# Kier73/Adaptive-Matrix-Solver

Measured on AMD Instinct MI355X. Metric: candidate-steps/sec, n=4096 dense eig pop=256, 1/2/4/8 GPUs vs CPU ref, higher is better.
Workload: dtype f64; 1 GPU; n=4096 dense non-Hermitian eig (complex128 Ginibre/sqrt(n)), initial_num_candidates=256, direct-LU InverseIterateSolver path; n=4096, pop=256, device= (gfx950:sramecc+:xnack-)

## Files before the change

adaptive_matrix_solver_amd/csrc/zgemm.hip:

```cpp
#include "common.h"
#include <cstdlib>

#ifndef MAUS_WC
#define MAUS_WC 8
#endif

namespace {

struct TCol { int x, y, z; };
__device__ __forceinline__ long tile_off(long rows, int col) { return ((long)(col >> 6) * rows << 6) + (col & 63); }

template <int BM, int BN, int BK, int WM, int WN, int BLAY, bool CONJA, bool CONJB, bool PIPE, int MINW, bool M3 = false, bool TILED = false>
__global__ void __launch_bounds__(64 * WM * WN, MINW)
zgemm_kernel(int M, int N, int K,
             const c128* __restrict__ Ag, long lda, long strideA,
             const c128* __restrict__ Bg, long ldb, long strideB,
             c128* __restrict__ Cg, long ldc, long strideC,
             double alpha, int beta, int tiles_n, int nwg,
             const int* __restrict__ a_rows, const int* __restrict__ c_rows, long rows_stride, TCol tcol)
{
    static_assert(!TILED || (BLAY == 0 && !CONJA && !CONJB && BK == 16), "tiled operands: plain layout, K-tiles of 16");
    constexpr int NT = 64 * WM * WN;
    constexpr int WTM = BM / WM, WTN = BN / WN;
    constexpr int MB = WTM / 16, NB = WTN / 16;
    constexpr int LDA_S = BM, LDB_S = BN;
    constexpr int A_PER = BM * BK / NT, B_PER = BN * BK / NT;
    static_assert(A_PER * NT == BM * BK && B_PER * NT == BN * BK, "tile/threads mismatch");

    constexpr int TILE_S = BK * LDA_S + BK * LDB_S;
    __shared__ c128 smem[(PIPE ? 2 : 1) * TILE_S];

    int bid = blockIdx.x;
    {
        int q = nwg >> 3, r = nwg & 7, xcd = bid & 7, idx = bid >> 3;
        bid = (xcd < r ? xcd * (q + 1) : r * (q + 1) + (xcd - r) * q) + idx;
    }
#ifndef MAUS_WC
#define MAUS_WC 8
#endif
    constexpr int WC = MAUS_WC;
    const int tiles_m = nwg / tiles_n;
    const int full = tiles_m * WC;
    int cb = bid / full, rem = bid - cb * full, wl = WC;
    const int ncb = (tiles_n + WC - 1) / WC;
    if (cb >= ncb - 1) { cb = ncb - 1; rem = bid - cb * full; wl = tiles_n - cb * WC; }
    const int tm = rem / wl, tn = cb * WC + (rem - tm * wl);
    const int m0 = tm * BM, n0 = tn * BN;
    const long batch = blockIdx.y;
    const c128* A = Ag + batch * strideA;
    const c128* B = Bg + batch * strideB;
    c128* C = Cg + batch * strideC;
    if (a_rows) a_rows += batch * rows_stride;
    if (c_rows) c_rows += batch * rows_stride;

    const int tid = threadIdx.x, lane = tid & 63, wave = tid >> 6;
    const int wm = wave / WN, wn = wave - wm * WN;

    d4 cre[MB][NB], cim[MB][NB], c3[M3 ? MB : 1][M3 ? NB : 1];
#pragma unroll
    for (int i = 0; i < MB; ++i)
#pragma unroll
        for (int j = 0; j < NB; ++j) {
            cre[i][j] = (d4){0, 0, 0, 0}; cim[i][j] = (d4){0, 0, 0, 0};
            if (M3) c3[i][j] = (d4){0, 0, 0, 0};
        }

    c128 ra[A_PER], rb[B_PER];

    const bool KEDGE = (K % BK) != 0;
    const c128* pa[A_PER];
    const c128* pb[B_PER];
#pragma unroll
    for (int i = 0; i < A_PER; ++i) {
        int r = tid / BK + i * (NT / BK);
        int gm = min(m0 + r, M - 1);
        pa[i] = A + (long)(a_rows ? a_rows[gm] : gm) * (TILED ? 64 : lda);
    }
#pragma unroll
    for (int i = 0; i < B_PER; ++i) {
        if (BLAY == 0) { int gn = min(n0 + tid % BN, N - 1); pb[i] = B + (TILED ? tile_off(ldb, tcol.z + gn) + (long)tcol.y * 64 : (long)gn); }
        else { int gn = min(n0 + tid / BK + i * (NT / BK), N - 1); pb[i] = B + (long)gn * ldb; }
    }
    const long ldb_e = TILED ? 64 : ldb;
    if (BLAY == 0) {
#pragma unroll
        for (int i = 0; i < B_PER; ++i) pb[i] += (long)(tid / BN + i * (NT / BN)) * ldb_e;
    }
    int kload = 0;
    auto load_tiles = [&](int k0) {
        kload = k0;
        const long ta = TILED ? tile_off(lda, tcol.x + k0) : 0;
#pragma unroll
        for (int i = 0; i < A_PER; ++i) {
            int gk = k0 + (tid & (BK - 1));
            if (TILED) ra[i] = pa[i][ta + (tid & (BK - 1))];
            else ra[i] = pa[i][KEDGE ? min(gk, K - 1) : gk];
        }
#pragma unroll
        for (int i = 0; i < B_PER; ++i) {
            if (BLAY == 0) {
                const int kr = tid / BN + i * (NT / BN);
                if (!KEDGE || TILED) rb[i] = pb[i][(long)k0 * ldb_e];
                else rb[i] = pb[i][(long)(min(k0 + kr, K - 1) - kr) * ldb];
            } else {
                int gk = k0 + (tid & (BK - 1));
                rb[i] = pb[i][KEDGE ? min(gk, K - 1) : gk];
            }
        }
    };
    auto store_tiles = [&](int buf) {
        c128* As = smem + buf * TILE_S;
        c128* Bs = As + BK * LDA_S;
#pragma unroll
        for (int i = 0; i < A_PER; ++i) {
            int k = tid & (BK - 1), r = tid / BK + i * (NT / BK);
            c128 v = ra[i];
            if (KEDGE && kload + k >= K) v = cmake(0.0, 0.0);
            if (CONJA) v.y = -v.y;
            As[k * LDA_S + (r ^ (k & 7))] = v;
        }
        if (BLAY == 0) {
#pragma unroll
            for (int i = 0; i < B_PER; ++i) {
                int n = tid % BN, k = tid / BN + i * (NT / BN);
                c128 v = rb[i];
                if (KEDGE && kload + k >= K) v = cmake(0.0, 0.0);
                if (CONJB) v.y = -v.y;
                Bs[k * LDB_S + (n ^ (k & 7))] = v;
            }
        } else {
#pragma unroll
            for (int i = 0; i < B_PER; ++i) {
                int k = tid & (BK - 1), r = tid / BK + i * (NT / BK);
                c128 v = rb[i];
                if (KEDGE && kload + k >= K) v = cmake(0.0, 0.0);
                if (CONJB) v.y = -v.y;
                Bs[k * LDB_S + (r ^ (k & 7))] = v;
            }
        }
    };

    const int nkt = (K + BK - 1) / BK;
    constexpr int KSTEPS = BK / 4;
    c128 fa[2][MB], fb[2][NB];
    auto read_frags = [&](int buf, int kk, int slot) {
        const c128* As = smem + buf * TILE_S;
        const c128* Bs = As + BK * LDA_S;
        const int krow = kk * 4 + (lane >> 4);
#pragma unroll
        for (int i = 0; i < MB; ++i) fa[slot][i] = As[krow * LDA_S + ((wm * WTM + i * 16 + (lane & 15)) ^ (krow & 7))];
#pragma unroll
        for (int j = 0; j < NB; ++j) fb[slot][j] = Bs[krow * LDB_S + ((wn * WTN + j * 16 + (lane & 15)) ^ (krow & 7))];
    };
    auto mfma_group = [&](int slot) {
        if (M3) {
            double as[MB], bs[NB];
#pragma unroll
            for (int i = 0; i < MB; ++i) as[i] = fa[slot][i].x + fa[slot][i].y;
#pragma unroll
            for (int j = 0; j < NB; ++j) bs[j] = fb[slot][j].x + fb[slot][j].y;
#pragma unroll
            for (int i = 0; i < MB; ++i)
#pragma unroll
                for (int j = 0; j < NB; ++j) {
                    cre[i][j] = __builtin_amdgcn_mfma_f64_16x16x4f64(fa[slot][i].x, fb[slot][j].x, cre[i][j], 0, 0, 0);
                    cim[i][j] = __builtin_amdgcn_mfma_f64_16x16x4f64(fa[slot][i].y, fb[slot][j].y, cim[i][j], 0, 0, 0);
                    c3[i][j] = __builtin_amdgcn_mfma_f64_16x16x4f64(as[i], bs[j], c3[i][j], 0, 0, 0);
                }
        } else {
#pragma unroll
            for (int i = 0; i < MB; ++i)
#pragma unroll
                for (int j = 0; j < NB; ++j) {
                    cre[i][j] = __builtin_amdgcn_mfma_f64_16x16x4f64(fa[slot][i].x, fb[slot][j].x, cre[i][j], 0, 0, 0);
                    cim[i][j] = __builtin_amdgcn_mfma_f64_16x16x4f64(fa[slot][i].x, fb[slot][j].y, cim[i][j], 0, 0, 0);
                }
#pragma unroll
            for (int i = 0; i < MB; ++i)
#pragma unroll
                for (int j = 0; j < NB; ++j) {
                    cre[i][j] = __builtin_amdgcn_mfma_f64_16x16x4f64(fa[slot][i].y, fb[slot][j].y, cre[i][j], 0, 0, 1);
                    cim[i][j] = __builtin_amdgcn_mfma_f64_16x16x4f64(fa[slot][i].y, fb[slot][j].x, cim[i][j], 0, 0, 0);
                }
        }
    };

    if (PIPE) {
        load_tiles(0);
        store_tiles(0);
        if (nkt > 1) load_tiles(BK);
        __syncthreads();
        for (int kt = 0; kt < nkt; ++kt) {
            const int buf = kt & 1;
            read_frags(buf, 0, 0);
#pragma unroll
            for (int kk = 0; kk < KSTEPS; ++kk) {
                if (kk + 1 < KSTEPS) read_frags(buf, kk + 1, (kk + 1) & 1);
                if (kk == 0 && kt + 1 < nkt) store_tiles(buf ^ 1);
                if (kk == 0 && kt + 2 < nkt) load_tiles((kt + 2) * BK);
                __builtin_amdgcn_sched_barrier(0);
                mfma_group(kk & 1);
                __builtin_amdgcn_sched_barrier(0);
            }
            __syncthreads();
        }
    } else {
        load_tiles(0);
        for (int kt = 0; kt < nkt; ++kt) {
            __syncthreads();
            store_tiles(0);
            __syncthreads();
            if (kt + 1 < nkt) load_tiles((kt + 1) * BK);
            read_frags(0, 0, 0);
#pragma unroll
            for (int kk = 0; kk < KSTEPS; ++kk) {
                if (kk + 1 < KSTEPS) read_frags(0, kk + 1, (kk + 1) & 1);
                mfma_group(kk & 1);
            }
        }
    }

#pragma unroll
    for (int i = 0; i < MB; ++i)
#pragma unroll
        for (int j = 0; j < NB; ++j) {
            const int gn = n0 + wn * WTN + j * 16 + (lane & 15);
            c128 cold[4];
            long off[4];
#pragma unroll
            for (int r = 0; r < 4; ++r) {
                const int gm = m0 + wm * WTM + i * 16 + (lane >> 4) + 4 * r;
                const int cm = min(gm, M - 1), cn = min(gn, N - 1);
                off[r] = TILED ? (long)(c_rows ? c_rows[cm] : cm) * 64 + tile_off(ldc, tcol.z + cn)
                               : (long)(c_rows ? c_rows[cm] : cm) * ldc + cn;
                cold[r] = cmake(0.0, 0.0);
                if (beta) cold[r] = C[off[r]];
            }
#pragma unroll
            for (int r = 0; r < 4; ++r) {
                const int gm = m0 + wm * WTM + i * 16 + (lane >> 4) + 4 * r;
                if (gm < M && gn < N) {
                    const double vr = M3 ? cre[i][j][r] - cim[i][j][r] : cre[i][j][r];
                    const double vi = M3 ? (c3[i][j][r] - cre[i][j][r]) - cim[i][j][r] : cim[i][j][r];
                    C[off[r]] = cmake(alpha * vr + cold[r].x, alpha * vi + cold[r].y);
                }
            }
        }
}

template <int NST, int MINW, int MB, int NB, bool TILED = false, int BLAY = 0, bool CONJA = false, bool CONJB = false>
__global__ void __launch_bounds__(256, MINW)
zgemm3m_dma_kernel(int M, int N, int K,
                   const c128* __restrict__ Ag, long lda, long strideA,
                   const c128* __restrict__ Bg, long ldb, long strideB,
                   c128* __restrict__ Cg, long ldc, long strideC,
                   double alpha, int beta, int tiles_n, int nwg,
                   const int* __restrict__ a_rows, const int* __restrict__ c_rows, long rows_stride, TCol tcol)
{
    constexpr int WN = 2, BM = 2 * 16 * MB, BN = WN * 16 * NB, BKS = 8;
    constexpr int A_ST = BM * BKS, B_ST = BKS * BN;
    constexpr int A_PW = BM / 32;
    constexpr int B_PW = BN / 32;
    constexpr int DMA_PW = A_PW + B_PW;
    __shared__ c128 smem[NST * (A_ST + B_ST)];

    int bid = blockIdx.x;
    {
        int q = nwg >> 3, r = nwg & 7, xcd = bid & 7, idx = bid >> 3;
        bid = (xcd < r ? xcd * (q + 1) : r * (q + 1) + (xcd - r) * q) + idx;
    }
    constexpr int WC = MAUS_WC;
    const int tiles_m = nwg / tiles_n;
    const int full = tiles_m * WC;
    int cb = bid / full, rem = bid - cb * full, wl = WC;
    const int ncb = (tiles_n + WC - 1) / WC;
    if (cb >= ncb - 1) { cb = ncb - 1; rem = bid - cb * full; wl = tiles_n - cb * WC; }
    const int tm = rem / wl, tn = cb * WC + (rem - tm * wl);
    const int m0 = tm * BM, n0 = tn * BN;
    const long batch = blockIdx.y;
    const c128* A = Ag + batch * strideA;
    const c128* B = Bg + batch * strideB;
    c128* C = Cg + batch * strideC;
    if (a_rows) a_rows += batch * rows_stride;
    if (c_rows) c_rows += batch * rows_stride;

    const int tid = threadIdx.x, lane = tid & 63, wave = tid >> 6;
    const int wm = wave / WN, wn = wave - wm * WN;

    const c128* srcA[A_PW];
#pragma unroll
    for (int j = 0; j < A_PW; ++j) {
        const int r = (A_PW * wave + j) * 8 + (lane >> 3);
        const int kk = (lane & 7) ^ ((r >> 1) & 7);
        const int gm = min(m0 + r, M - 1);
        srcA[j] = A + (long)(a_rows ? a_rows[gm] : gm) * (TILED ? 64 : lda) + kk;
    }
    static_assert(!(TILED && BLAY), "tiled operands: plain layout only");
    const c128* srcB[B_PW];
    const long ldb_e = TILED ? 64 : ldb;
#pragma unroll
    for (int j = 0; j < B_PW; ++j) {
        if (BLAY == 0) {
            const int e = (B_PW * wave + j) * 64 + lane;
            const int gn = min(n0 + (e % BN), N - 1);
            srcB[j] = B + (long)(e / BN) * ldb_e + (TILED ? tile_off(ldb, tcol.z + gn) + (long)tcol.y * 64 : (long)gn);
        } else {
            const int r = (B_PW * wave + j) * 8 + (lane >> 3);
            const int kk = (lane & 7) ^ ((r >> 1) & 7);
            srcB[j] = B + (long)min(n0 + r, N - 1) * ldb + kk;
        }
    }

    auto issue = [&](int st, int k0) {
        c128* As = smem + st * (A_ST + B_ST);
        c128* Bs = As + A_ST;
        const long ta = TILED ? tile_off(lda, tcol.x + k0) : (long)k0;
#pragma unroll
        for (int j = 0; j < A_PW; ++j)
            __builtin_amdgcn_global_load_lds((const void*)(srcA[j] + ta), (__attribute__((address_space(3))) void*)(As + (A_PW * wave + j) * 64), 16, 0, 0);
#pragma unroll
        for (int j = 0; j < B_PW; ++j)
            __builtin_amdgcn_global_load_lds((const void*)(srcB[j] + (BLAY ? (long)k0 : (long)k0 * ldb_e)), (__attribute__((address_space(3))) void*)(Bs + (B_PW * wave + j) * 64), 16, 0, 0);
    };

    d4 cre[MB][NB], cim[MB][NB], c3[MB][NB];
#pragma unroll
    for (int i = 0; i < MB; ++i)
#pragma unroll
        for (int j = 0; j < NB; ++j) { cre[i][j] = (d4){0, 0, 0, 0}; cim[i][j] = (d4){0, 0, 0, 0}; c3[i][j] = (d4){0, 0, 0, 0}; }

    const int nst = K / BKS;
#pragma unroll
    for (int s = 0; s < NST - 1; ++s) if (s < nst) issue(s, s * BKS);

    const int arow0 = wm * 16 * MB + (lane & 15);
    const int bcol0 = wn * 16 * NB + (lane & 15);
    const int q = lane >> 4;
    for (int t = 0; t < nst; ++t) {
        if (NST >= 3 && t + NST - 2 < nst) asm volatile("s_waitcnt vmcnt(%0)" :: "n"((NST - 2) * DMA_PW) : "memory");
        else asm volatile("s_waitcnt vmcnt(0)" ::: "memory");
        __builtin_amdgcn_s_barrier();
        asm volatile("" ::: "memory");
        const c128* As = smem + (t % NST) * (A_ST + B_ST);
        const c128* Bs = As + A_ST;
        c128 fa[2][MB], fb[2][NB];
#pragma unroll
        for (int ks = 0; ks < 2; ++ks) {
            const int k = ks * 4 + q;
#pragma unroll
            for (int i = 0; i < MB; ++i) {
                const int r = arow0 + i * 16;
                fa[ks][i] = As[r * BKS + (k ^ ((r >> 1) & 7))];
            }
#pragma unroll
            for (int j = 0; j < NB; ++j) {
                const int cn = bcol0 + j * 16;
                fb[ks][j] = BLAY ? Bs[cn * BKS + (k ^ ((cn >> 1) & 7))] : Bs[k * BN + cn];
            }
        }
        if (t + NST - 1 < nst) issue((t + NST - 1) % NST, (t + NST - 1) * BKS);
#pragma unroll
        for (int ks = 0; ks < 2; ++ks) {
            double as[MB], bs[NB];
#pragma unroll
            for (int i = 0; i < MB; ++i) as[i] = CONJA ? fa[ks][i].x - fa[ks][i].y : fa[ks][i].x + fa[ks][i].y;
#pragma unroll
            for (int j = 0; j < NB; ++j) bs[j] = CONJB ? fb[ks][j].x - fb[ks][j].y : fb[ks][j].x + fb[ks][j].y;
#pragma unroll
            for (int i = 0; i < MB; ++i)
#pragma unroll
                for (int j = 0; j < NB; ++j) {
                    cre[i][j] = __builtin_amdgcn_mfma_f64_16x16x4f64(fa[ks][i].x, fb[ks][j].x, cre[i][j], 0, 0, 0);
                    cim[i][j] = __builtin_amdgcn_mfma_f64_16x16x4f64(fa[ks][i].y, fb[ks][j].y, cim[i][j], 0, 0, 0);
                    c3[i][j] = __builtin_amdgcn_mfma_f64_16x16x4f64(as[i], bs[j], c3[i][j], 0, 0, 0);
                }
        }
    }
    constexpr double S2 = (CONJA != CONJB) ? -1.0 : 1.0;

#pragma unroll
    for (int i = 0; i < MB; ++i)
#pragma unroll
        for (int j = 0; j < NB; ++j) {
            const int gn = n0 + wn * 16 * NB + j * 16 + (lane & 15);
            c128 cold[4];
            long off[4];
#pragma unroll
            for (int r = 0; r < 4; ++r) {
                const int gm = m0 + wm * 16 * MB + i * 16 + (lane >> 4) + 4 * r;
                const int cm = min(gm, M - 1), cn = min(gn, N - 1);
                off[r] = TILED ? (long)(c_rows ? c_rows[cm] : cm) * 64 + tile_off(ldc, tcol.z + cn)
                               : (long)(c_rows ? c_rows[cm] : cm) * ldc + cn;
                cold[r] = cmake(0.0, 0.0);
                if (beta) cold[r] = C[off[r]];
            }
#pragma unroll
            for (int r = 0; r < 4; ++r) {
                const int gm = m0 + wm * 16 * MB + i * 16 + (lane >> 4) + 4 * r;
                if (gm < M && gn < N) {
                    const double vr = cre[i][j][r] - S2 * cim[i][j][r];
                    const double vi = (c3[i][j][r] - cre[i][j][r]) - S2 * cim[i][j][r];
                    C[off[r]] = cmake(alpha * vr + cold[r].x, alpha * vi + cold[r].y);
                }
            }
        }
}

template <int NST, int MINW, int MB, int NB, bool TILED = false, int BLAY = 0, bool CONJA = false, bool CONJB = false>
void launch_dma(hipStream_t st, int M, int N, int K, const c128* A, long lda, long sA, const c128* B, long ldb, long sB,
                c128* C, long ldc, long sC, double alpha, int beta, int batch, int, bool, bool,
                const int* a_rows, const int* c_rows, long rows_stride, TCol tcol = TCol{0, 0, 0})
{
    constexpr int BM = 32 * MB, BN = 32 * NB;
    int tiles_m = (M + BM - 1) / BM, tiles_n = (N + BN - 1) / BN;
    int nwg = tiles_m * tiles_n;
    hipLaunchKernelGGL((zgemm3m_dma_kernel<NST, MINW, MB, NB, TILED, BLAY, CONJA, CONJB>), dim3(nwg, batch), dim3(256), 0, st,
                       M, N, K, A, lda, sA, B, ldb, sB, C, ldc, sC, alpha, beta, tiles_n, nwg, a_rows, c_rows, rows_stride, tcol);
}

template <int BLAY, bool CONJA, bool CONJB>
void launch_dma_pop(hipStream_t st, int M, int N, int K, const c128* A, long lda, long sA, const c128* B, long ldb, long sB,
                    c128* C, long ldc, long sC, double alpha, int beta, int batch, int blay, bool conja, bool conjb,
                    const int* a_rows, const int* c_rows, long rows_stride)
{
    if (M >= 1536 && N >= 1536) launch_dma<2, 3, 2, 2, false, BLAY, CONJA, CONJB>(st, M, N, K, A, lda, sA, B, ldb, sB, C, ldc, sC, alpha, beta, batch, blay, conja, conjb, a_rows, c_rows, rows_stride);
    else launch_dma<2, 5, 2, 1, false, BLAY, CONJA, CONJB>(st, M, N, K, A, lda, sA, B, ldb, sB, C, ldc, sC, alpha, beta, batch, blay, conja, conjb, a_rows, c_rows, rows_stride);
}

template <int BM, int BN, int BK, int WM, int WN, bool PIPE, int MINW>
void launch_cfg(hipStream_t st, int M, int N, int K, const c128* A, long lda, long sA, const c128* B, long ldb, long sB,
                c128* C, long ldc, long sC, double alpha, int beta, int batch, int blay, bool conja, bool conjb,
                const int* a_rows, const int* c_rows, long rows_stride)
{
    int tiles_m = (M + BM - 1) / BM, tiles_n = (N + BN - 1) / BN;
    int nwg = tiles_m * tiles_n;
    dim3 grid(nwg, batch), block(64 * WM * WN);
#define LAUNCH(BL, CA, CB) hipLaunchKernelGGL((zgemm_kernel<BM, BN, BK, WM, WN, BL, CA, CB, PIPE, MINW>), grid, block, 0, st, \
        M, N, K, A, lda, sA, B, ldb, sB, C, ldc, sC, alpha, beta, tiles_n, nwg, a_rows, c_rows, rows_stride, TCol{0, 0, 0})
    if (blay == 0) {
        if (!conja && !conjb) LAUNCH(0, false, false);
        else if (!conja && conjb) LAUNCH(0, false, true);
        else if (conja && !conjb) LAUNCH(0, true, false);
        else LAUNCH(0, true, true);
    } else {
        if (!conja && !conjb) LAUNCH(1, false, false);
        else if (!conja && conjb) LAUNCH(1, false, true);
        else if (conja && !conjb) LAUNCH(1, true, false);
        else LAUNCH(1, true, true);
    }
#undef LAUNCH
}

template <int BM, int BN, int BK, int WM, int WN, bool PIPE = false, int MINW = 4, bool M3 = false, bool TILED = false>
void launch_lu_only(hipStream_t st, int M, int N, int K, const c128* A, long lda, long sA, const c128* B, long ldb, long sB,
                    c128* C, long ldc, long sC, double alpha, int beta, int batch, int, bool, bool,
                    const int* a_rows, const int* c_rows, long rows_stride, TCol tcol = TCol{0, 0, 0})
{
    int tiles_m = (M + BM - 1) / BM, tiles_n = (N + BN - 1) / BN;
    int nwg = tiles_m * tiles_n;
    hipLaunchKernelGGL((zgemm_kernel<BM, BN, BK, WM, WN, 0, false, false, PIPE, MINW, M3, TILED>), dim3(nwg, batch), dim3(64 * WM * WN), 0, st,
                       M, N, K, A, lda, sA, B, ldb, sB, C, ldc, sC, alpha, beta, tiles_n, nwg, a_rows, c_rows, rows_stride, tcol);
}

}

void maus_zgemm_launch_rows(hipStream_t st, int M, int N, int K, const c128* A, long lda, long sA,
                            const c128* B, long ldb, long sB, c128* C, long ldc, long sC,
                            double alpha, int beta, int batch, int blay, bool conja, bool conjb,
                            const int* a_rows, const int* c_rows, long rows_stride)
{
    if (M <= 0 || N <= 0 || batch <= 0) return;
#define ARGS st, M, N, K, A, lda, sA, B, ldb, sB, C, ldc, sC, alpha, beta, batch, blay, conja, conjb, a_rows, c_rows, rows_stride
    constexpr int DMA_KMIN = 64;
    if (blay == 0 && !conja && !conjb) {
        if (N <= 16) { launch_lu_only<128, 16, 16, 4, 1>(ARGS); return; }
        if (M <= 16) { launch_lu_only<16, 128, 16, 1, 4, false, 3>(ARGS); return; }
        if (M > 32 && (K % 8) == 0 && K >= DMA_KMIN) {
            if (M >= 1536 && N >= 1536) launch_dma<2, 3, 2, 2>(ARGS);
            else launch_dma<2, 5, 2, 1>(ARGS);
            return;
        }
        if (M <= 32) { launch_lu_only<32, 64, 16, 1, 4, false, 4, true>(ARGS); return; }
        launch_lu_only<64, 32, 16, 2, 2, false, 4, true>(ARGS); return;
    }
    if (M > 32 && (K % 8) == 0 && K >= DMA_KMIN) {
        if (blay == 1 && !conja && !conjb) { launch_dma_pop<1, false, false>(ARGS); return; }
        if (blay == 1 && conja && !conjb) { launch_dma_pop<1, true, false>(ARGS); return; }
        if (blay == 1 && !conja && conjb) { launch_dma_pop<1, false, true>(ARGS); return; }
        if (blay == 0 && conja && !conjb) { launch_dma_pop<0, true, false>(ARGS); return; }
        if (blay == 0 && !conja && conjb) { launch_dma_pop<0, false, true>(ARGS); return; }
    }
    const long t64 = (long)((M + 63) / 64) * ((N + 63) / 64) * batch;
    const int tile = (t64 >= 512) ? 0 : ((long)((M + 31) / 32) * ((N + 63) / 64) * batch >= 512 ? 1 : 2);
    if (tile == 1) { launch_cfg<32, 64, 16, 1, 4, false, 4>(ARGS); return; }
    if (tile == 2) { launch_cfg<32, 32, 16, 2, 2, false, 4>(ARGS); return; }
    launch_cfg<64, 64, 16, 2, 2, false, 3>(ARGS);
#undef ARGS
}

void maus_zgemm_launch_lu(hipStream_t st, int M, int N, int K, const c128* H, const c128* U, c128* Hc, long nrows, long stride,
                          int acol, int brow, int ccol, int batch, const int* rows, long rows_stride)
{
    if (M <= 0 || N <= 0 || K <= 0 || batch <= 0) return;
    constexpr int dma_kmin = 64;
    const TCol tc{acol, brow, ccol};
#define ARGS st, M, N, K, H, nrows, stride, U, nrows, stride, Hc, nrows, stride, -1.0, 1, batch, 0, false, false, rows, rows, rows_stride, tc
    if (N <= 16) { launch_lu_only<128, 16, 16, 4, 1, false, 4, false, true>(ARGS); return; }
    if (M <= 16) { launch_lu_only<16, 128, 16, 1, 4, false, 3, false, true>(ARGS); return; }
    if (M > 32 && (K % 8) == 0 && K >= dma_kmin) {
        if (M >= 1536 && N >= 1536) launch_dma<2, 3, 2, 2, true>(ARGS);
        else launch_dma<2, 5, 2, 1, true>(ARGS);
        return;
    }
    if (M <= 32) { launch_lu_only<32, 64, 16, 1, 4, false, 4, true, true>(ARGS); return; }
    launch_lu_only<64, 32, 16, 2, 2, false, 4, true, true>(ARGS);
#undef ARGS
}

void maus_zgemm_launch_idx(hipStream_t st, int M, int N, int K, const c128* A, long lda, long sA,
                           const c128* B, long ldb, long sB, c128* C, long ldc, long sC,
                           double alpha, int beta, int batch, int blay, bool conja, bool conjb,
                           const int* a_rows, const int* c_rows)
{
    maus_zgemm_launch_rows(st, M, N, K, A, lda, sA, B, ldb, sB, C, ldc, sC, alpha, beta, batch, blay, conja, conjb, a_rows, c_rows, 0);
}

void maus_zgemm_launch(hipStream_t st, int M, int N, int K, const c128* A, long lda, long sA,
                       const c128* B, long ldb, long sB, c128* C, long ldc, long sC,
                       double alpha, int beta, int batch, int blay, bool conja, bool conjb)
{
    maus_zgemm_launch_idx(st, M, N, K, A, lda, sA, B, ldb, sB, C, ldc, sC, alpha, beta, batch, blay, conja, conjb, nullptr, nullptr);
}
```

Baseline: 375.5 candidate-steps/s.

## Add large-tile LU trailing-update ZGEMM with 32-bit offset addressing

Adds a new DMA-path configuration for the tiled LU trailing-update GEMM, selected when M,N are large, K>=256 and the batched tile count is high (or forced by an env var). For these large-register-tile variants, global loads use a scalar base plus 32-bit per-lane offsets, and LDS fragment reads use precomputed addresses. The aim is fewer VGPRs and address-arithmetic instructions and more data reuse per tile. The trade-off is possible occupancy loss from the larger tile and a risk of 32-bit offset overflow on very large matrices.

```diff
diff --git a/adaptive_matrix_solver_amd/csrc/zgemm.hip b/adaptive_matrix_solver_amd/csrc/zgemm.hip
--- a/adaptive_matrix_solver_amd/csrc/zgemm.hip
+++ b/adaptive_matrix_solver_amd/csrc/zgemm.hip
@@ -1,5 +1,7 @@
 #include "common.h"
+#include <cstdio>
 #include <cstdlib>
+#include <cstring>
 
 #ifndef MAUS_WC
 #define MAUS_WC 8
@@ -287,7 +289,32 @@
     const int tid = threadIdx.x, lane = tid & 63, wave = tid >> 6;
     const int wm = wave / WN, wn = wave - wm * WN;
 
-    const c128* srcA[A_PW];
+    constexpr bool OFF32 = TILED && BLAY == 0 && MB * NB >= 8;
+    constexpr int B_CP = OFF32 ? BN / 64 : 1;
+    static_assert(!OFF32 || (BN % 64 == 0 && B_PW % B_CP == 0), "OFF32: whole 64-column pieces");
+    const c128* srcA[OFF32 ? 1 : A_PW];
+    const c128* srcB[OFF32 ? 1 : B_PW];
+    unsigned offA[OFF32 ? A_PW : 1], offB[OFF32 ? B_CP : 1];
+    const int wave_u = __builtin_amdgcn_readfirstlane(wave);
+    const long ldb_e = TILED ? 64 : ldb;
+    static_assert(!(TILED && BLAY), "tiled operands: plain layout only");
+    if constexpr (OFF32) {
+#pragma unroll
+        for (int j = 0; j < A_PW; ++j) {
+            const int r = (A_PW * wave + j) * 8 + (lane >> 3);
+            const int kk = (lane & 7) ^ ((r >> 1) & 7);
+            const int gm = min(m0 + r, M - 1);
+            offA[j] = (unsigned)((a_rows ? a_rows[gm] : gm) * 64 + kk) * 16u;
+        }
+        const int ct0 = (tcol.z + n0) >> 6;
+#pragma unroll
+        for (int c = 0; c < B_CP; ++c) {
+            const int col = tcol.z + min(n0 + c * 64 + lane, N - 1);
+            offB[c] = (unsigned)(((col >> 6) - ct0) * (int)ldb * 64 + (col & 63)) * 16u;
+        }
+        srcA[0] = A;
+        srcB[0] = B + ((long)ct0 * ldb << 6) + (long)(tcol.y + (B_PW / B_CP) * wave_u) * 64;
+    } else {
 #pragma unroll
     for (int j = 0; j < A_PW; ++j) {
         const int r = (A_PW * wave + j) * 8 + (lane >> 3);
@@ -295,9 +322,6 @@
         const int gm = min(m0 + r, M - 1);
         srcA[j] = A + (long)(a_rows ? a_rows[gm] : gm) * (TILED ? 64 : lda) + kk;
     }
-    static_assert(!(TILED && BLAY), "tiled operands: plain layout only");
-    const c128* srcB[B_PW];
-    const long ldb_e = TILED ? 64 : ldb;
 #pragma unroll
     for (int j = 0; j < B_PW; ++j) {
         if (BLAY == 0) {
@@ -310,11 +334,31 @@
             srcB[j] = B + (long)min(n0 + r, N - 1) * ldb + kk;
         }
     }
+    }
 
     auto issue = [&](int st, int k0) {
         c128* As = smem + st * (A_ST + B_ST);
         c128* Bs = As + A_ST;
         const long ta = TILED ? tile_off(lda, tcol.x + k0) : (long)k0;
+        if constexpr (OFF32) {
+            const char* ba = (const char*)(srcA[0] + ta);
+            const char* bb = (const char*)(srcB[0] + (long)k0 * 64);
+            asm volatile("" : "+s"(ba), "+s"(bb));
+#pragma unroll
+            for (int j = 0; j < A_PW; ++j) {
+                unsigned o = offA[j];
+                asm volatile("" : "+v"(o));
+                __builtin_amdgcn_global_load_lds((const void*)(ba + o), (__attribute__((address_space(3))) void*)(As + (A_PW * wave_u + j) * 64), 16, 0, 0);
+            }
+#pragma unroll
+            for (int j = 0; j < B_PW; ++j) {
+                unsigned o = offB[j % B_CP];
+                asm volatile("" : "+v"(o));
+                if (j && j % B_CP == 0) { bb += 1024; asm volatile("" : "+s"(bb)); }
+                __builtin_amdgcn_global_load_lds((const void*)(bb + o), (__attribute__((address_space(3))) void*)(Bs + (B_PW * wave_u + j) * 64), 16, 0, 0);
+            }
+            return;
+        }
 #pragma unroll
         for (int j = 0; j < A_PW; ++j)
             __builtin_amdgcn_global_load_lds((const void*)(srcA[j] + ta), (__attribute__((address_space(3))) void*)(As + (A_PW * wave + j) * 64), 16, 0, 0);
@@ -336,6 +380,15 @@
     const int arow0 = wm * 16 * MB + (lane & 15);
     const int bcol0 = wn * 16 * NB + (lane & 15);
     const int q = lane >> 4;
+    typedef double lds_d2_t __attribute__((ext_vector_type(2)));
+    typedef __attribute__((address_space(3))) const lds_d2_t lds_d2;
+    unsigned ra[2] = {0, 0}, rb = 0;
+    if constexpr (OFF32) {
+        static_assert(NST == 2, "OFF32: two stages");
+        const unsigned sb = (unsigned)(unsigned long)(__attribute__((address_space(3))) void*)smem;
+        for (int ks = 0; ks < 2; ++ks) ra[ks] = sb + 16u * (arow0 * BKS + ((ks * 4 + q) ^ ((arow0 >> 1) & 7)));
+        rb = sb + 16u * (A_ST + q * BN + bcol0);
+    }
     for (int t = 0; t < nst; ++t) {
         if (NST >= 3 && t + NST - 2 < nst) asm volatile("s_waitcnt vmcnt(%0)" :: "n"((NST - 2) * DMA_PW) : "memory");
         else asm volatile("s_waitcnt vmcnt(0)" ::: "memory");
@@ -350,12 +403,14 @@
 #pragma unroll
             for (int i = 0; i < MB; ++i) {
                 const int r = arow0 + i * 16;
-                fa[ks][i] = As[r * BKS + (k ^ ((r >> 1) & 7))];
+                if constexpr (OFF32) { const lds_d2_t v = *(lds_d2*)(unsigned long)(ra[ks] + (t & 1) * (16u * (A_ST + B_ST)) + 16u * (i * 16 * BKS)); fa[ks][i] = cmake(v.x, v.y); }
+                else fa[ks][i] = As[r * BKS + (k ^ ((r >> 1) & 7))];
             }
 #pragma unroll
             for (int j = 0; j < NB; ++j) {
                 const int cn = bcol0 + j * 16;
-                fb[ks][j] = BLAY ? Bs[cn * BKS + (k ^ ((cn >> 1) & 7))] : Bs[k * BN + cn];
+                if constexpr (OFF32) { const lds_d2_t v = *(lds_d2*)(unsigned long)(rb + (t & 1) * (16u * (A_ST + B_ST)) + 16u * (ks * 4 * BN + j * 16)); fb[ks][j] = cmake(v.x, v.y); }
+                else fb[ks][j] = BLAY ? Bs[cn * BKS + (k ^ ((cn >> 1) & 7))] : Bs[k * BN + cn];
             }
         }
         if (t + NST - 1 < nst) issue((t + NST - 1) % NST, (t + NST - 1) * BKS);
@@ -462,6 +517,23 @@
                        M, N, K, A, lda, sA, B, ldb, sB, C, ldc, sC, alpha, beta, tiles_n, nwg, a_rows, c_rows, rows_stride, tcol);
 }
 
+#ifndef MAUS_LU_LT_MIN
+#define MAUS_LU_LT_MIN 1024
+#endif
+int lu_tile_mode()
+{
+    static const int mode = [] {
+        const char* e = getenv("MAUS_LU_TILE");
+        if (!e || !*e) return 0;
+        if (!strcmp(e, "128x64")) return 2;
+        if (!strcmp(e, "64x64")) return 3;
+        fprintf(stderr, "MAUS_LU_TILE=%s: expected 64x64 or 128x64\n", e);
+        abort();
+        return 0;
+    }();
+    return mode;
+}
+
 }
 
 void maus_zgemm_launch_rows(hipStream_t st, int M, int N, int K, const c128* A, long lda, long sA,
@@ -508,8 +580,11 @@
     if (N <= 16) { launch_lu_only<128, 16, 16, 4, 1, false, 4, false, true>(ARGS); return; }
     if (M <= 16) { launch_lu_only<16, 128, 16, 1, 4, false, 3, false, true>(ARGS); return; }
     if (M > 32 && (K % 8) == 0 && K >= dma_kmin) {
-        if (M >= 1536 && N >= 1536) launch_dma<2, 3, 2, 2, true>(ARGS);
-        else launch_dma<2, 5, 2, 1, true>(ARGS);
+        const int tile = lu_tile_mode();
+        const long tiles = (long)((M + 127) / 128) * ((N + 63) / 64) * batch;
+        if (M >= MAUS_LU_LT_MIN && N >= MAUS_LU_LT_MIN && (tile == 2 || (tile == 0 && K >= 256 && tiles >= 4096))) { launch_dma<2, 2, 4, 2, true>(ARGS); return; }
+        if (M >= 1536 && N >= 1536) { launch_dma<2, 3, 2, 2, true>(ARGS); return; }
+        launch_dma<2, 5, 2, 1, true>(ARGS);
         return;
     }
     if (M <= 32) { launch_lu_only<32, 64, 16, 1, 4, false, 4, true, true>(ARGS); return; }
```

Result: faster. 383.2 candidate-steps/s (median of 6 runs) (+2.1%).
